# mct10/Speech-Vecalign

Measured on AMD Instinct MI355X. Metric: aligned doc-pairs/sec, higher is better.
Workload: dtype bf16; 1 GPU; synthetic 4096x4096 d=1024 bf16 embeddings, 4 overlap layers/side, 10 alignment types, band 14, coarse-to-fine (max_size_full_dp=300), 1024 doc-pairs per GPU per step; pipeline=1, N=4096, M=4096, d=1024, overlaps=4, parallelism=dp1 (pairs sharded, no collective)

## Files before the change

### speech-vecalign_amd/csrc/svx_api.hip

```cpp
#include <stdarg.h>
#include <stdio.h>
#include <stdlib.h>
#include <string.h>

#include <chrono>
#include <functional>
#include <memory>
#include <type_traits>
#include <vector>

#include "svx_common.h"

static char g_err[512] = "";

int svx_fail(svx_ctx* ctx, int code, const char* fmt, ...) {
    char* dst = ctx ? ctx->err : g_err;
    va_list ap;
    va_start(ap, fmt);
    vsnprintf(dst, 512, fmt, ap);
    va_end(ap);
    return code;
}

static const char* kStageNames[] = {"pyr0",       "pyrN",     "pyr_aux",      "knob_scoresN", "knob",      "dense_costs",
// ... 809 lines not shown
    if (bump.off > H.arena_bytes) {
        SVX_HIP(ctx, hipDeviceSynchronize());
        if (H.arena) SVX_HIP(ctx, hipFree(H.arena));
        H.arena = nullptr;
        H.arena_bytes = 0;
        const size_t want = bump.off + bump.off / 16 + (1 << 20);
        hipError_t e = hipMalloc(&H.arena, want);
        if (e != hipSuccess) return svx_fail(ctx, SVX_ERR_NOMEM, "scratch arena: hipMalloc(%zu) failed: %s", want, hipGetErrorString(e));
        H.arena_bytes = want;
    }
    const size_t desc_bytes = (size_t)n_pairs * sizeof(SvxPairDev);
    if (desc_bytes > H.pinned_cap) {
        SVX_HIP(ctx, hipDeviceSynchronize());
        if (H.pinned) SVX_HIP(ctx, hipHostFree(H.pinned));
        H.pinned = nullptr;
        H.pinned_cap = 0;
        SVX_HIP(ctx, hipHostMalloc(reinterpret_cast<void**>(&H.pinned), desc_bytes + desc_bytes / 8, hipHostMallocDefault));
        H.pinned_cap = desc_bytes + desc_bytes / 8;
    }
    char* base = H.arena;
    const char* ulo = reinterpret_cast<const char*>(1);
    const char* uhi = reinterpret_cast<const char*>(bump.off + 1);
    auto patch = [&](auto& ptr) {
        const char* v = reinterpret_cast<const char*>(ptr);
        if (v >= ulo && v < uhi) ptr = reinterpret_cast<typename std::remove_reference<decltype(ptr)>::type>(base + (v - ulo));
    };
    for (int p = 0; p < n_pairs; p++) {
        SvxPairDev& P = host[p];
        const svx_pair& in = pairs[p];
        for (int l = 0; l <= P.L; l++) {
            SvxLevel& Lv = P.lev[l];
            for (int s = 0; s < 2; s++) {
                patch(Lv.P[s]); patch(Lv.part[s]); patch(Lv.mean[s]); patch(Lv.rbar[s]); patch(Lv.inv[s]);
                if (!(l == 0 && P.norm_override[s])) patch(Lv.nrm[s]);
            }
            patch(Lv.kscore); patch(Lv.korder); patch(Lv.kys); patch(Lv.kstart);
            if (!in.del_pen) patch(Lv.pen);
            patch(Lv.path); patch(Lv.path_len); patch(Lv.cstart); patch(Lv.nchunks); patch(Lv.costs); patch(Lv.boff); patch(Lv.csum); patch(Lv.xp); patch(Lv.yp); patch(Lv.bpk);
            patch(Lv.boff_out);
            if (l > 0) { patch(Lv.align); patch(Lv.scores); patch(Lv.n_align); }
        }
        patch(P.dcost);
        patch(P.ddot);
        patch(P.dbp);
        patch(P.t_lo); patch(P.t_cnt); patch(P.t_pref); patch(P.t_flag);
    }
    H.dpairs = reinterpret_cast<SvxPairDev*>(base + o_desc);
    return SVX_OK;
}

struct Op {
    double us;
    int stage;
    std::function<int()> fn;
};

static int run_op(svx_ctx* ctx, const Op& op, hipStream_t st) {
    hipStream_t keep = ctx->stream;
    ctx->stream = st;
    int rc;
    if (op.stage < 0) {
        rc = op.fn();
    } else {
        StageScope sc(ctx, op.stage);
        rc = op.fn();
    }
    ctx->stream = keep;
    return rc;
}

static int next_event(svx_ctx* ctx, hipEvent_t* out) {
    svx_ctx_ext* cx = X(ctx);
    if (cx->ev_pool.size() < 256) {
        hipEvent_t e;
        SVX_HIP(ctx, hipEventCreateWithFlags(&e, hipEventDisableTiming));
        cx->ev_pool.push_back(e);
        *out = e;
        return SVX_OK;
    }
    *out = cx->ev_pool[cx->ev_next++ % cx->ev_pool.size()];
    return SVX_OK;
}

static void front_ops(svx_ctx* ctx, HalfState& H, std::vector<Op>& ops, int split) {
    svx_ctx_ext* cx = X(ctx);
    HalfState* h = &H;
    const BatchParams& bp = H.bp;
    const int np = H.n_pairs, d = bp.d, dtype = bp.dtype;
    const double waves = (double)((np + 1023) / 1024);
    const int parts = (split > 1 && np >= 16 * split) ? split : 1;
    struct Evs { hipEvent_t pass[SVX_MAX_LEVELS][8]; };
    auto evs = std::make_shared<Evs>();
    ops.push_back({0.0, -1, [=]() -> int {
        SVX_HIP(ctx, hipEventRecord(cx->side_fork, ctx->stream));
        SVX_HIP(ctx, hipStreamWaitEvent(cx->side, cx->side_fork, 0));
        SVX_HIP(ctx, hipStreamWaitEvent(cx->helper, cx->side_fork, 0));
        return SVX_OK;
    }});
    static const bool early_sort = getenv("SVX_SORT_EARLY") != nullptr;
    auto sort_op = [=]() -> int {
        hipStream_t main_stream = ctx->stream;
        static const bool inline_sort = getenv("SVX_SORT_INLINE") != nullptr;
        if (parts > 1 && !inline_sort && !early_sort) SVX_HIP(ctx, hipStreamWaitEvent(cx->side, evs->pass[0][parts - 1], 0));
        ctx->stream = inline_sort ? main_stream : cx->side;
        int rc;
        {
            StageScope sc(ctx, S_KNOB_SORT);
            rc = svxl_knob_scores(ctx, h->dpairs, np, h->maxL, h->max_kn, h->max_n0, dtype, d, 0);
        }
        ctx->stream = main_stream;
        if (rc) return rc;
        SVX_HIP(ctx, hipEventRecord(cx->side_join, inline_sort ? main_stream : cx->side));
        return SVX_OK;
    };
    if (parts == 1 || early_sort) ops.push_back({0.0, -1, sort_op});
    for (int l = 0; l <= H.maxL; l++) {
        for (int q = 0; q < parts; q++) {
            const int lo = (int)((long long)np * q / parts), hi = (int)((long long)np * (q + 1) / parts);
            const double aux_us = (l == 0 ? 700.0 * waves : 250.0) / parts;
            if (parts == 1) {
                ops.push_back({aux_us, S_PYR_AUX, [=]() { return svxl_pyramid_level(ctx, h->dpairs, np, l, dtype, d, h->max_nblk[l], h->max_ksum, 0); }});
                ops.push_back({H.b_pyr[l] / (l == 0 ? 4.9e6 : 5.3e6), l == 0 ? S_PYR0 : (l == 1 ? S_PYR1 : S_PYRN),
                               [=]() { return svxl_pyramid_level(ctx, h->dpairs, np, l, dtype, d, h->max_nblk[l], h->max_ksum, 1); }});
                continue;
            }
            ops.push_back({H.b_pyr[l] / (l == 0 ? 4.9e6 : 5.3e6) / parts, l == 0 ? S_PYR0 : (l == 1 ? S_PYR1 : S_PYRN), [=]() -> int {
                hipStream_t main_stream = ctx->stream;
                int rc;
                if (l == 0 && q == 0) {
                    StageScope sc(ctx, S_PYR_AUX);
                    if ((rc = svxl_pyramid_level(ctx, h->dpairs + lo, hi - lo, l, dtype, d, h->max_nblk[l], h->max_ksum, 0))) return rc;
                } else {
                    if (l > 0) SVX_HIP(ctx, hipStreamWaitEvent(cx->helper, evs->pass[l - 1][q], 0));
                    ctx->stream = cx->helper;
                    {
                        StageScope sc(ctx, S_PYR_AUX);
                        rc = svxl_pyramid_level(ctx, h->dpairs + lo, hi - lo, l, dtype, d, h->max_nblk[l], h->max_ksum, 0);
                    }
                    ctx->stream = main_stream;
                    if (rc) return rc;
                    hipEvent_t aux_done;
                    if ((rc = next_event(ctx, &aux_done))) return rc;
                    SVX_HIP(ctx, hipEventRecord(aux_done, cx->helper));
                    SVX_HIP(ctx, hipStreamWaitEvent(main_stream, aux_done, 0));
                }
                if ((rc = svxl_pyramid_level(ctx, h->dpairs + lo, hi - lo, l, dtype, d, h->max_nblk[l], h->max_ksum, 1))) return rc;
                if ((rc = next_event(ctx, &evs->pass[l][q]))) return rc;
                SVX_HIP(ctx, hipEventRecord(evs->pass[l][q], main_stream));
                return SVX_OK;
            }});
        }
        if (parts > 1 && l == 0 && !early_sort) ops.push_back({0.0, -1, sort_op});
    }
    if (!bp.straight) {
        ops.push_back({H.dense_cells * 2.7e-5, S_DENSE_COSTS, [=]() -> int {
            int rc = svxl_dense_costs_batch(ctx, h->dpairs, np, h->max_ds0, h->max_ds1, dtype, d);
            if (rc) return rc;
            return svxl_knob_from_dots(ctx, h->dpairs, np, h->max_kn);
        }});
    }
    if (H.maxL >= 1) {
        ops.push_back({H.b_knobN / 16.5e6, S_KNOB_SCORES, [=]() -> int {
            SVX_HIP(ctx, hipStreamWaitEvent(ctx->stream, cx->side_join, 0));
            return svxl_knob_scores(ctx, h->dpairs, np, h->maxL, h->max_kn, h->max_n0, dtype, d, 1);
        }});
    }
    ops.push_back({H.b_knob0 / 8.5e6, S_KNOB_SCORES0, [=]() -> int {
        SVX_HIP(ctx, hipStreamWaitEvent(ctx->stream, cx->side_join, 0));
        return svxl_knob_scores(ctx, h->dpairs, np, h->maxL, h->max_kn, h->max_n0, dtype, d, 2);
    }});
}

struct Seg {
    std::vector<Op> lb;
    bool has_s = false;
    Op s;
};

static void chain_segs(svx_ctx* ctx, HalfState& H, std::vector<Seg>& segs) {
    HalfState* h = &H;
    const BatchParams bp = H.bp;
    const int np = H.n_pairs, d = bp.d, dtype = bp.dtype, W = bp.W, B = bp.B;
    const double waves = (double)((np + 1023) / 1024);
    Seg cur;
    cur.lb.push_back({(np * (H.maxL + 1) * 0.21 < 300.0 ? 300.0 : np * (H.maxL + 1) * 0.21), S_KNOB,
                      [=]() { return svxl_del_penalty_batch(ctx, h->dpairs, np, h->maxL + 1, bp.frac); }});
    if (!bp.straight)
        cur.lb.push_back({(H.max_ds0 + H.max_ds1) * 1.7 * waves, S_DENSE_DP, [=]() { return svxl_dense_stage_batch(ctx, h->dpairs, np, h->max_ds0); }});
    const int first_depth = H.maxL > 0 ? H.maxL - 1 : 0;
    for (int depth = first_depth; depth >= 0; depth--) {
        const SvxTypes ty = depth == 0 ? bp.tfinal : bp.t11;
        int lim = 0, tamax = 0;
        if (!bp.tiles) svxl_band2_limits(ty, W, depth, dtype, d, &lim, &tamax);
        const int maxA = H.max_A[depth];
        const int src_rows = (H.maxL > 0 && !H.any_L0) ? maxA / 2 + 8 : maxA;
        cur.lb.push_back({maxA * 0.08 * waves + 60.0, depth == 0 ? S_PATH0 : S_PATH, [=]() {
            return svxl_search_path_batch(ctx, h->dpairs, np, depth, maxA, src_rows, lim, tamax);
        }});
        cur.has_s = true;
        if (bp.tiles) {
            cur.s = {1.0e4, S_TILES, [=]() {
                int* tk = reinterpret_cast<int*>(h->arena + h->o_tickets);
                float* planes = h->b_planes ? reinterpret_cast<float*>(h->arena + h->o_planes) : nullptr;
                return svxl_band_tiles_batch(ctx, h->dpairs, np, ty, W, dtype, h->max_tnd, tk, tk + (size_t)h->max_tnd * np + 1, planes);
            }};
        } else {
            cur.s = {H.b_bc[depth] / 4.0e6, depth == 0 ? S_BAND_COSTS0 : S_BAND_COSTSN, [=]() {
                return svxl_band_costs2_batch(ctx, h->dpairs, np, depth, maxA, ty, W, dtype, d);
            }};
        }
        segs.push_back(cur);
        cur = Seg();
        if (!bp.tiles)
            cur.lb.push_back({maxA * (0.21 + 0.054 * (ty.n > 1 ? ty.n : 0)) * waves, depth == 0 ? S_BAND_DP0 : S_BAND_DPN,
                              [=]() { return svxl_sparse_dp_batch(ctx, h->dpairs, np, depth, ty, B); }});
        cur.lb.push_back({maxA * 0.27 * waves, depth == 0 ? S_TRACEBACK0 : S_TRACEBACK, [=]() { return svxl_sparse_traceback_batch(ctx, h->dpairs, np, depth, B, maxA, bp.packable ? 1 : 0); }});
    }
    segs.push_back(cur);
}

static int ensure_streams(svx_ctx* ctx) {
    svx_ctx_ext* cx = X(ctx);
    if (!cx->side_ready) {
        int prio_lo = 0, prio_hi = 0;
        SVX_HIP(ctx, hipDeviceGetStreamPriorityRange(&prio_lo, &prio_hi));
        SVX_HIP(ctx, hipStreamCreateWithPriority(&cx->side, hipStreamNonBlocking, prio_lo));
        SVX_HIP(ctx, hipStreamCreateWithPriority(&cx->helper, hipStreamNonBlocking, prio_hi));
        SVX_HIP(ctx, hipEventCreateWithFlags(&cx->side_fork, hipEventDisableTiming));
        SVX_HIP(ctx, hipEventCreateWithFlags(&cx->side_join, hipEventDisableTiming));
        cx->side_ready = true;
    }
    if (!cx->chain_ready) {
        int prio_lo = 0, prio_hi = 0;
        SVX_HIP(ctx, hipDeviceGetStreamPriorityRange(&prio_lo, &prio_hi));
        SVX_HIP(ctx, hipStreamCreateWithPriority(&cx->chain, hipStreamNonBlocking, prio_hi));
        cx->chain_ready = true;
    }
    for (int h = 0; h < 2; h++) {
        if (!cx->half[h].front_done) SVX_HIP(ctx, hipEventCreateWithFlags(&cx->half[h].front_done, hipEventDisableTiming));
        if (!cx->half[h].chain_done) SVX_HIP(ctx, hipEventCreateWithFlags(&cx->half[h].chain_done, hipEventDisableTiming));
        if (!cx->half[h].upload_done) SVX_HIP(ctx, hipEventCreateWithFlags(&cx->half[h].upload_done, hipEventDisableTiming));
    }
    return SVX_OK;
}

static int run_interleaved(svx_ctx* ctx, HalfState* front, HalfState* chain, bool beside) {
    svx_ctx_ext* cx = X(ctx);
    hipStream_t A = ctx->stream, Bst = beside ? cx->chain : ctx->stream;
    std::vector<Op> fops;
    std::vector<Seg> segs;
    if (front) {
        if (front->chain_done_valid) SVX_HIP(ctx, hipStreamWaitEvent(A, front->chain_done, 0));
        {
            StageScope sc(ctx, S_SETUP);
            if (front->upload_valid) SVX_HIP(ctx, hipEventSynchronize(front->upload_done));
            memcpy(front->pinned, front->host.data(), (size_t)front->n_pairs * sizeof(SvxPairDev));
            SVX_HIP(ctx, hipMemcpyAsync(front->dpairs, front->pinned, (size_t)front->n_pairs * sizeof(SvxPairDev), hipMemcpyHostToDevice, A));
            SVX_HIP(ctx, hipEventRecord(front->upload_done, A));
            front->upload_valid = true;
            hipLaunchKernelGGL(k_init_batch, dim3(front->n_pairs), dim3(64), 0, A, front->dpairs);
            SVX_LAUNCH_CHECK(ctx, "k_init_batch");
            if (front->bp.around) {
                int rc = svxl_prior_ingest_batch(ctx, front->dpairs, front->n_pairs);
                if (rc) return rc;
            }
            if (front->bp.nsamp == 0) {
                for (int p = 0; p < front->n_pairs; p++)
                    for (int l = 0; l <= front->host[p].L; l++)
                        for (int s = 0; s < 2; s++)
                            SVX_HIP(ctx, hipMemsetAsync(front->host[p].lev[l].rbar[s], 0, (size_t)front->bp.d * sizeof(float), A));
            }
        }
        static const int split_env = [] { const char* e = getenv("SVX_PIPE_SPLIT"); const int v = e ? atoi(e) : 2; return v >= 1 && v <= 8 ? v : 2; }();
        front_ops(ctx, *front, fops, beside ? split_env : 1);
    }
    if (chain) chain_segs(ctx, *chain, segs);
    int rc;
    size_t fi = 0;
    if (chain && beside) SVX_HIP(ctx, hipStreamWaitEvent(Bst, chain->front_done, 0));
    for (size_t g = 0; g < segs.size(); g++) {
        double need = 0.0;
        for (const Op& op : segs[g].lb) {
            if ((rc = run_op(ctx, op, Bst))) return rc;
            need += op.us;
        }
        hipEvent_t lb_done = nullptr;
        if (beside) {
            if ((rc = next_event(ctx, &lb_done))) return rc;
            SVX_HIP(ctx, hipEventRecord(lb_done, Bst));
        }
        if (!segs[g].has_s) break;
        double acc = 0.0;
        need = need * 1.25 + 50.0;
        while (beside && fi < fops.size() && acc < need) {
            if ((rc = run_op(ctx, fops[fi], A))) return rc;
            acc += fops[fi].us;
            fi++;
        }
        if (beside) SVX_HIP(ctx, hipStreamWaitEvent(A, lb_done, 0));
        if ((rc = run_op(ctx, segs[g].s, A))) return rc;
        if (beside) {
            hipEvent_t s_done;
            if ((rc = next_event(ctx, &s_done))) return rc;
            SVX_HIP(ctx, hipEventRecord(s_done, A));
            SVX_HIP(ctx, hipStreamWaitEvent(Bst, s_done, 0));
        }
    }
    for (; fi < fops.size(); fi++)
        if ((rc = run_op(ctx, fops[fi], A))) return rc;
    if (front) {
        SVX_HIP(ctx, hipEventRecord(front->front_done, A));
        front->chain_pending = true;
    }
    if (chain) {
        SVX_HIP(ctx, hipEventRecord(chain->chain_done, Bst));
        chain->chain_done_valid = true;
        chain->chain_pending = false;
    }
    return SVX_OK;
}

extern "C" int svx_flush(svx_ctx* ctx) {
    if (!ctx) return SVX_ERR_ARG;
    svx_ctx_ext* cx = X(ctx);
    bool any = false;
    for (int h = 0; h < 2; h++) any = any || cx->half[h].chain_pending || cx->half[h].chain_done_valid;
    if (!any) return SVX_OK;
    SVX_HIP(ctx, hipSetDevice(ctx->device));
    int rc;
    for (int h = 0; h < 2; h++)
        if (cx->half[h].chain_pending && (rc = run_interleaved(ctx, nullptr, &cx->half[h], true))) return rc;
    for (int h = 0; h < 2; h++)
        if (cx->half[h].chain_done_valid) SVX_HIP(ctx, hipStreamWaitEvent(ctx->stream, cx->half[h].chain_done, 0));
    return SVX_OK;
}

static int align_impl(svx_ctx* ctx, const svx_align_params* prm, const svx_pair* pairs, const svx_prior* priors, int n_pairs) {
// ... 185 lines not shown
```

### speech-vecalign_amd/csrc/svx_costs.hip

```cpp
#include <stdlib.h>

#include "svx_common.h"
#include "svx_slab.h"

namespace {

constexpr int RS = 144;

template <typename E>
struct Mma;
template <>
struct Mma<ElemBF16> {
    static constexpr int KS = 64, NK = 2, KSTEP_BYTES = 64;
    using frag = uint4;
    __device__ static __forceinline__ int lane_off(int lane) { return (lane & 15) * RS + 16 * (lane >> 4); }
    __device__ static __forceinline__ frag load(const char* p) { return *reinterpret_cast<const uint4*>(p); }
    __device__ static __forceinline__ void mma(f32x4_t& acc, const frag& a, const frag& b) {
        acc = __builtin_amdgcn_mfma_f32_16x16x32_bf16(__builtin_bit_cast(bf16x8_t, a), __builtin_bit_cast(bf16x8_t, b), acc, 0, 0, 0);
    }
};
template <>
struct Mma<ElemF16> {
    static constexpr int KS = 64, NK = 2, KSTEP_BYTES = 64;
    using frag = uint4;
    __device__ static __forceinline__ int lane_off(int lane) { return (lane & 15) * RS + 16 * (lane >> 4); }
    __device__ static __forceinline__ frag load(const char* p) { return *reinterpret_cast<const uint4*>(p); }
    __device__ static __forceinline__ void mma(f32x4_t& acc, const frag& a, const frag& b) {
        acc = __builtin_amdgcn_mfma_f32_16x16x32_f16(__builtin_bit_cast(f16x8_t, a), __builtin_bit_cast(f16x8_t, b), acc, 0, 0, 0);
    }
};
template <>
struct Mma<ElemF32> {
    static constexpr int KS = 32, NK = 8, KSTEP_BYTES = 16;
    using frag = float;
    __device__ static __forceinline__ int lane_off(int lane) { return (lane & 15) * RS + 4 * (lane >> 4); }
    __device__ static __forceinline__ frag load(const char* p) { return *reinterpret_cast<const float*>(p); }
    __device__ static __forceinline__ void mma(f32x4_t& acc, const frag& a, const frag& b) {
        acc = __builtin_amdgcn_mfma_f32_16x16x4f32(a, b, acc, 0, 0, 0);
    }
};

template <typename E>
__device__ __forceinline__ void stage_slab(char* slab, const char* const* rowptr, int nrows, int k0, int d, int tid,
                                           int nthreads) {
    using S = typename E::storage;
    const int npieces = nrows * 8;
    for (int q = tid; q < npieces; q += nthreads) {
        const int r = q >> 3, p = q & 7;
        const char* ptr = rowptr[r];
        const int kel = k0 + p * E::VEC;
        uint4 v = make_uint4(0, 0, 0, 0);
        if (ptr != nullptr && kel < d) v = *reinterpret_cast<const uint4*>(ptr + (size_t)kel * sizeof(S));
        *reinterpret_cast<uint4*>(slab + r * RS + p * 16) = v;
    }
}

struct DenseArgs {
    const void* v0;
    const void* v1;
    int s0, s1, d;
    const float* inv0;
    const float* inv1;
    const float* n0;
    const float* n1;
    int mul0, mul1;
    float* costs;
    float* dots;
};

constexpr int DT = 64;
template <typename E>
__device__ void dense_block(const DenseArgs& g, int bx, int by, char* smem) {
    using S = typename E::storage;
    const int tid = threadIdx.x, lane = tid & 63, wave = tid >> 6;
    const char** rowptr = reinterpret_cast<const char**>(smem);
    char* slab = smem + 2 * DT * sizeof(char*);
    const int x0 = bx * DT, y0 = by * DT;
    if (tid < 2 * DT) {
        const int side = tid >= DT, loc = tid - side * DT;
        const int gi = (side ? y0 : x0) + loc;
        const int nn = side ? g.s1 : g.s0;
        const char* base = reinterpret_cast<const char*>(side ? g.v1 : g.v0);
        rowptr[tid] = (gi < nn) ? base + (size_t)gi * g.d * sizeof(S) : nullptr;
    }
    f32x4_t acc[2][2];
#pragma unroll
    for (int i = 0; i < 2; i++)
#pragma unroll
        for (int j = 0; j < 2; j++) acc[i][j] = (f32x4_t){0.f, 0.f, 0.f, 0.f};
    const int xt = wave >> 1, yt = wave & 1;
    for (int k0 = 0; k0 < g.d; k0 += Mma<E>::KS) {
        __syncthreads();
        stage_slab<E>(slab, rowptr, 2 * DT, k0, g.d, tid, blockDim.x);
        __syncthreads();
        const char* ap = slab + xt * 32 * RS + Mma<E>::lane_off(lane);
        const char* bp = slab + (DT + yt * 32) * RS + Mma<E>::lane_off(lane);
#pragma unroll
        for (int ks = 0; ks < Mma<E>::NK; ks++) {
            const typename Mma<E>::frag a0 = Mma<E>::load(ap + ks * Mma<E>::KSTEP_BYTES);
            const typename Mma<E>::frag a1 = Mma<E>::load(ap + 16 * RS + ks * Mma<E>::KSTEP_BYTES);
            const typename Mma<E>::frag b0 = Mma<E>::load(bp + ks * Mma<E>::KSTEP_BYTES);
            const typename Mma<E>::frag b1 = Mma<E>::load(bp + 16 * RS + ks * Mma<E>::KSTEP_BYTES);
            Mma<E>::mma(acc[0][0], a0, b0);
            Mma<E>::mma(acc[0][1], a0, b1);
            Mma<E>::mma(acc[1][0], a1, b0);
            Mma<E>::mma(acc[1][1], a1, b1);
        }
    }
#pragma unroll
    for (int i = 0; i < 2; i++)
#pragma unroll
        for (int j = 0; j < 2; j++) {
            const int y = y0 + yt * 32 + j * 16 + (lane & 15);
#pragma unroll
            for (int r = 0; r < 4; r++) {
                const int x = x0 + xt * 32 + i * 16 + (lane >> 4) * 4 + r;
                if (x < g.s0 && y < g.s1) {
                    float sumx = acc[i][j][r];
                    if (g.inv0) sumx = sumx * g.inv0[x] * g.inv1[y];
                    float c = cost_formula(sumx, 1, 1, g.n0[x], g.n1[y]);
                    c = (c * (float)g.mul0) * (float)g.mul1;
                    g.costs[(size_t)x * g.s1 + y] = c;
                    if (g.dots) g.dots[(size_t)x * g.s1 + y] = sumx;
                }
            }
        }
}

template <typename E>
__global__ __launch_bounds__(256) void k_dense_costs(DenseArgs g) {
    extern __shared__ __attribute__((aligned(16))) char smem[];
    dense_block<E>(g, blockIdx.x, blockIdx.y, smem);
}

template <typename E, bool LV0>
__global__ __launch_bounds__(256) void k_dense_costs_batch(const SvxPairDev* __restrict__ pairs) {
    extern __shared__ __attribute__((aligned(16))) char smem[];
    const SvxPairDev& P = pairs[blockIdx.z];
    if ((P.L == 0) != LV0) return;
    const SvxLevel& Lv = P.lev[P.L];
    DenseArgs g;
    g.s0 = Lv.n[0];
    g.s1 = Lv.n[1];
    if ((int)blockIdx.x * DT >= g.s0 || (int)blockIdx.y * DT >= g.s1) return;
    g.d = P.d;
    g.v0 = LV0 ? P.v[0] : (const void*)Lv.P[0];
    g.v1 = LV0 ? P.v[1] : (const void*)Lv.P[1];
    g.inv0 = LV0 ? Lv.inv[0] : nullptr;
    g.inv1 = LV0 ? Lv.inv[1] : nullptr;
    g.n0 = Lv.nrm[0];
    g.n1 = Lv.nrm[1];
    g.mul0 = 1;
    g.mul1 = 1;
    g.costs = P.dcost;
    g.dots = LV0 ? nullptr : P.ddot;
    dense_block<E>(g, blockIdx.x, blockIdx.y, smem);
}

template <typename E, int NCH>
__device__ __forceinline__ float row_dot(const typename E::storage* a, const typename E::storage* b, int d, int lane) {
    float s = 0.f;
#pragma unroll
    for (int c = 0; c < NCH; c++) {
        const int col = (c * SVX_WAVE + lane) * E::VEC;
        if (col < d) {
            float x[E::VEC], y[E::VEC];
            load_piece<E>(a + col, x);
            load_piece<E>(b + col, y);
#pragma unroll
            for (int i = 0; i < E::VEC; i++) s += x[i] * y[i];
        }
    }
    return wave_sum(s);
}

struct ScoreArgs {
    const void* v1;
    const void* v2;
    const float* inv1;
    const float* inv2;
    const float* n1;
    const float* n2;
    const int* xx;
    const int* yy;
    int64_t n;
    int rows1, rows2, d;
    float* out;
};

template <typename E, int NCH>
__device__ void score_block(const ScoreArgs& g, int64_t first, int64_t stride) {
    using S = typename E::storage;
    const int lane = threadIdx.x & 63;
    for (int64_t i = first; i < g.n; i += stride) {
        int xi = g.xx[i], yi = g.yy[i];
        xi = xi < 0 ? 0 : (xi >= g.rows1 ? g.rows1 - 1 : xi);
        yi = yi < 0 ? 0 : (yi >= g.rows2 ? g.rows2 - 1 : yi);
        float dot = row_dot<E, NCH>(reinterpret_cast<const S*>(g.v1) + (size_t)xi * g.d,
                                    reinterpret_cast<const S*>(g.v2) + (size_t)yi * g.d, g.d, lane);
        if (lane == 0) {
            if (g.inv1) dot = dot * g.inv1[xi] * g.inv2[yi];
            const float den = g.n1[xi] + g.n2[yi];
            g.out[i] = (float)((2.0 * (1.0 - (double)dot)) / (double)den);
        }
    }
}

template <typename E, int NCH>
__global__ __launch_bounds__(256) void k_score_path(ScoreArgs g) {
    score_block<E, NCH>(g, (int64_t)blockIdx.x * 4 + (threadIdx.x >> 6), (int64_t)gridDim.x * 4);
}

template <int NT>
__device__ __forceinline__ void knob_sort_block(const int* __restrict__ kx, const int* __restrict__ ky, int kn, int n, int m,
                                                int* __restrict__ korder, int* __restrict__ kys, int* __restrict__ kstart,
                                                int* cnt, int* part, size_t lds_bytes) {
    const int tid = threadIdx.x, lane = tid & 63, wave = tid >> 6;
    const bool staged = ((size_t)n + 1 + (size_t)kn) * sizeof(int) <= lds_bytes;
    int* ord = cnt + n + 1;
    for (int i = tid; i < n; i += NT) cnt[i] = 0;
    __syncthreads();
    for (int i = tid; i < kn; i += NT) {
        int x = kx[i];
        x = x < 0 ? 0 : (x >= n ? n - 1 : x);
        atomicAdd(&cnt[x], 1);
    }
    __syncthreads();
    const int per = (n + NT - 1) / NT;
    const int lo = tid * per < n ? tid * per : n, hi = (lo + per) < n ? (lo + per) : n;
    int sum = 0;
    for (int i = lo; i < hi; i++) sum += cnt[i];
    int inc = sum;
#pragma unroll
    for (int o = 1; o < 64; o <<= 1) {
        const int t = __shfl_up(inc, o, 64);
        if (lane >= o) inc += t;
    }
    if (lane == 63) part[wave] = inc;
    __syncthreads();
    int run = inc - sum;
    for (int w = 0; w < wave; w++) run += part[w];
    for (int i = lo; i < hi; i++) {
        const int v = cnt[i];
        cnt[i] = run;
        kstart[i] = run;
        run += v;
    }
    if (tid == 0) kstart[n] = kn;
    __syncthreads();
    if (staged) {
        for (int i = tid; i < kn; i += NT) {
            int x = kx[i];
            x = x < 0 ? 0 : (x >= n ? n - 1 : x);
            ord[atomicAdd(&cnt[x], 1)] = i;
        }
        __syncthreads();
        for (int p = tid; p < kn; p += NT) {
            const int i = ord[p];
            int y = ky[i];
            y = y < 0 ? 0 : (y >= m ? m - 1 : y);
            korder[p] = i;
            kys[p] = y;
        }
        return;
    }
    for (int i = tid; i < kn; i += NT) {
        int x = kx[i];
        x = x < 0 ? 0 : (x >= n ? n - 1 : x);
        const int pos = atomicAdd(&cnt[x], 1);
        int y = ky[i];
        y = y < 0 ? 0 : (y >= m ? m - 1 : y);
        korder[pos] = i;
        kys[pos] = y;
    }
}

template <int NT>
__global__ __launch_bounds__(NT) void k_knob_sort(const SvxPairDev* __restrict__ pairs, unsigned lds_bytes) {
    extern __shared__ __attribute__((aligned(16))) char smem[];
    __shared__ int part[NT / 64];
    const SvxPairDev& P = pairs[blockIdx.y];
    const int level = blockIdx.x;
    if (level > P.L) return;
    if (P.L >= 1 && level == P.L) return;
    const SvxLevel& Lv = P.lev[level];
    knob_sort_block<NT>(Lv.kx, Lv.ky, Lv.kn, Lv.n[0], Lv.n[1], Lv.korder, Lv.kys, Lv.kstart, reinterpret_cast<int*>(smem), part,
                        lds_bytes);
}

template <int NT>
__global__ __launch_bounds__(NT) void k_knob_sort_plain(const int* __restrict__ kx, const int* __restrict__ ky, int kn, int n, int m,
                                                        int* __restrict__ korder, int* __restrict__ kys, int* __restrict__ kstart,
                                                        unsigned lds_bytes) {
    extern __shared__ __attribute__((aligned(16))) char smem[];
    __shared__ int part[NT / 64];
    knob_sort_block<NT>(kx, ky, kn, n, m, korder, kys, kstart, reinterpret_cast<int*>(smem), part, lds_bytes);
}

constexpr int KNOB_PF = 2;

template <typename E, int NCH, bool LV0>
__global__ __launch_bounds__(256) void k_knob_scores(const SvxPairDev* __restrict__ pairs, int nlev, int bpt) {
    using S = typename E::storage;
    constexpr int EPL = NCH * E::VEC;
    const unsigned wg = xcd_remap(blockIdx.x, gridDim.x);
    const int task = wg / bpt, blk = wg % bpt;
    const SvxPairDev& P = pairs[task / nlev];
    const int level = task % nlev + (LV0 ? 0 : 1);
    if (level > P.L) return;
    if (!LV0 && level == P.L) return;
    const SvxLevel& Lv = P.lev[level];
    const int lane = threadIdx.x & 63;
    const int n = Lv.n[0], d = P.d;
    const S* v1 = LV0 ? reinterpret_cast<const S*>(P.v[0]) : reinterpret_cast<const S*>(Lv.P[0]);
    const S* v2 = LV0 ? reinterpret_cast<const S*>(P.v[1]) : reinterpret_cast<const S*>(Lv.P[1]);
    const float* inv1 = LV0 ? Lv.inv[0] : nullptr;
    const float* inv2 = LV0 ? Lv.inv[1] : nullptr;
    for (int x = blk * 4 + (threadIdx.x >> 6); x < n; x += bpt * 4) {
        const int s0 = gld(Lv.kstart + x), s1 = gld(Lv.kstart + x + 1);
        if (s0 >= s1) continue;
        float xr[EPL];
#pragma unroll
        for (int c = 0; c < NCH; c++) {
            const int col = (c * SVX_WAVE + lane) * E::VEC;
            if (col < d) {
                gload_piece<E>(v1 + (size_t)x * d + col, xr + c * E::VEC);
            } else {
#pragma unroll
                for (int i = 0; i < E::VEC; i++) xr[c * E::VEC + i] = 0.f;
            }
        }
        const float nx = gld(Lv.nrm[0] + x);
        const float ix = LV0 ? gld(inv1 + x) : 1.0f;
        constexpr int PF = KNOB_PF;
        const int ns = s1 - s0;
        for (int cb = 0; cb < ns; cb += SVX_WAVE) {
            const int cn = min(SVX_WAVE, ns - cb);
            const int ys_l = lane < cn ? gld(Lv.kys + s0 + cb + lane) : 0;
            const int is_l = lane < cn ? gld(Lv.korder + s0 + cb + lane) : 0;
            const float nrm_l = lane < cn ? gld(Lv.nrm[1] + ys_l) : 0.f;
            const float inv_l = (LV0 && lane < cn) ? gld(inv2 + ys_l) : 1.f;
            float dots_l = 0.f;
            uint4 yraw[PF][NCH];
#pragma unroll
            for (int u = 0; u < PF; u++) {
                const int yu = __builtin_amdgcn_readlane(ys_l, u);
#pragma unroll
                for (int c = 0; c < NCH; c++) {
                    const int col = (c * SVX_WAVE + lane) * E::VEC;
                    yraw[u][c] = (u < cn && col < d) ? gld16(v2 + (size_t)yu * d + col) : make_uint4(0, 0, 0, 0);
                }
            }
            for (int base = 0; base < cn; base += PF) {
#pragma unroll
                for (int u = 0; u < PF; u++) {
                    const int k = base + u;
                    if (k >= cn) break;
                    float dot = 0.f;
#pragma unroll
                    for (int c = 0; c < NCH; c++) {
                        float yr[E::VEC];
                        decode_piece<E>(yraw[u][c], yr);
#pragma unroll
                        for (int e = 0; e < E::VEC; e++) dot += xr[c * E::VEC + e] * yr[e];
                    }
                    if (k + PF < cn) {
                        const int yn = __builtin_amdgcn_readlane(ys_l, k + PF);
#pragma unroll
                        for (int c = 0; c < NCH; c++) {
                            const int col = (c * SVX_WAVE + lane) * E::VEC;
                            yraw[u][c] = col < d ? gld16(v2 + (size_t)yn * d + col) : make_uint4(0, 0, 0, 0);
                        }
                    }
                    dot = wave_sum(dot);
                    dots_l = lane == k ? dot : dots_l;
                }
            }
            if (lane < cn) {
                float dot = dots_l;
                if (LV0) dot = dot * ix * inv_l;
                const float den = nx + nrm_l;
                gst(Lv.kscore + is_l, (float)((2.0 * (1.0 - (double)dot)) / (double)den));
            }
        }
    }
}

template <typename E, int NCH, bool LV0>
__global__ __launch_bounds__(256) void k_knob_scores_unsorted(const SvxPairDev* __restrict__ pairs) {
    const SvxPairDev& P = pairs[blockIdx.z];
    const int level = (int)blockIdx.y + (LV0 ? 0 : 1);
    if (level > P.L) return;
    if (!LV0 && level == P.L) return;
    const SvxLevel& Lv = P.lev[level];
    ScoreArgs g;
    g.v1 = LV0 ? P.v[0] : (const void*)Lv.P[0];
    g.v2 = LV0 ? P.v[1] : (const void*)Lv.P[1];
    g.inv1 = LV0 ? Lv.inv[0] : nullptr;
    g.inv2 = LV0 ? Lv.inv[1] : nullptr;
    g.n1 = Lv.nrm[0];
    g.n2 = Lv.nrm[1];
    g.xx = Lv.kx;
    g.yy = Lv.ky;
    g.n = Lv.kn;
    g.rows1 = Lv.n[0];
    g.rows2 = Lv.n[1];
    g.d = P.d;
    g.out = Lv.kscore;
    score_block<E, NCH>(g, (int64_t)blockIdx.x * 4 + (threadIdx.x >> 6), (int64_t)gridDim.x * 4);
}

__global__ __launch_bounds__(256) void k_knob_from_dots(const SvxPairDev* __restrict__ pairs) {
    const SvxPairDev& P = pairs[blockIdx.y];
    if (P.L < 1) return;
    const SvxLevel& Lv = P.lev[P.L];
    const int n = Lv.n[0], m = Lv.n[1];
    for (int i = blockIdx.x * 256 + threadIdx.x; i < Lv.kn; i += gridDim.x * 256) {
        int x = Lv.kx[i], y = Lv.ky[i];
        x = x < 0 ? 0 : (x >= n ? n - 1 : x);
        y = y < 0 ? 0 : (y >= m ? m - 1 : y);
        const float dot = P.ddot[(size_t)x * m + y];
        const float den = Lv.nrm[0][x] + Lv.nrm[1][y];
        Lv.kscore[i] = (float)((2.0 * (1.0 - (double)dot)) / (double)den);
    }
}

inline int nch_f32(int d) {
    int c = (d + 255) / 256;
    return c <= 1 ? 1 : c <= 2 ? 2 : c <= 4 ? 4 : 8;
}
inline int nch_16(int d) {
    int c = (d + 511) / 512;
    return c <= 1 ? 1 : c <= 2 ? 2 : 4;
}

constexpr size_t DENSE_SMEM = 2 * DT * sizeof(char*) + 2 * DT * RS;

}

int svxl_dense_costs(svx_ctx* ctx, const float* v0, int s0, const float* v1, int s1, int d, const float* n0,
                     const float* n1, int mul0, int mul1, float* costs) {
    if (s0 <= 0 || s1 <= 0) return SVX_OK;
    DenseArgs g{v0, v1, s0, s1, d, nullptr, nullptr, n0, n1, mul0, mul1, costs, nullptr};
    hipLaunchKernelGGL(k_dense_costs<ElemF32>, dim3((s0 + DT - 1) / DT, (s1 + DT - 1) / DT), dim3(256), DENSE_SMEM, ctx->stream, g);
    SVX_LAUNCH_CHECK(ctx, "k_dense_costs");
    return SVX_OK;
}

int svxl_dense_costs_batch(svx_ctx* ctx, const SvxPairDev* pairs, int n_pairs, int max_s0, int max_s1, int dtype, int d) {
    (void)d;
    if (n_pairs <= 0 || max_s0 <= 0 || max_s1 <= 0) return SVX_OK;
    dim3 grid((max_s0 + DT - 1) / DT, (max_s1 + DT - 1) / DT, n_pairs);
    hipLaunchKernelGGL((k_dense_costs_batch<ElemF32, false>), grid, dim3(256), DENSE_SMEM, ctx->stream, pairs);
    if (dtype == SVX_F32)
        hipLaunchKernelGGL((k_dense_costs_batch<ElemF32, true>), grid, dim3(256), DENSE_SMEM, ctx->stream, pairs);
    else if (dtype == SVX_F16)
        hipLaunchKernelGGL((k_dense_costs_batch<ElemF16, true>), grid, dim3(256), DENSE_SMEM, ctx->stream, pairs);
    else
        hipLaunchKernelGGL((k_dense_costs_batch<ElemBF16, true>), grid, dim3(256), DENSE_SMEM, ctx->stream, pairs);
    SVX_LAUNCH_CHECK(ctx, "k_dense_costs_batch");
    return SVX_OK;
}

int svxl_score_path(svx_ctx* ctx, const int* xx, const int* yy, int64_t n, const float* n1, const float* n2,
                    const float* v1, int rows1, const float* v2, int rows2, int d, float* out) {
    if (n <= 0) return SVX_OK;
    ScoreArgs g{v1, v2, nullptr, nullptr, n1, n2, xx, yy, n, rows1, rows2, d, out};
    int64_t nb = (n + 3) / 4;
    if (nb > 16384) nb = 16384;
#define M(N) hipLaunchKernelGGL((k_score_path<ElemF32, N>), dim3((unsigned)nb), dim3(256), 0, ctx->stream, g)
    switch (nch_f32(d)) {
        case 1: M(1); break;
        case 2: M(2); break;
        case 4: M(4); break;
        default: M(8); break;
    }
#undef M
    SVX_LAUNCH_CHECK(ctx, "k_score_path");
    return SVX_OK;
}

int svxl_knob_from_dots(svx_ctx* ctx, const SvxPairDev* pairs, int n_pairs, int max_kn) {
    if (n_pairs <= 0 || max_kn <= 0) return SVX_OK;
    int nb = (max_kn + 255) / 256;
    if (nb > 16) nb = 16;
    hipLaunchKernelGGL(k_knob_from_dots, dim3(nb, n_pairs), dim3(256), 0, ctx->stream, pairs);
    SVX_LAUNCH_CHECK(ctx, "k_knob_from_dots");
    return SVX_OK;
}

constexpr size_t KNOB_SORT_HIST_LDS = 150 * 1024;
constexpr size_t KNOB_SORT_STAGE_LDS = SVX_KNOB_SORT_STAGE_LDS;
static_assert(KNOB_SORT_STAGE_LDS >= KNOB_SORT_HIST_LDS, "a launch sized for staging must still hold the longest histogram");

static size_t knob_sort_lds(int max_n0, int max_kn) {
    const size_t want = ((size_t)max_n0 + 1 + (size_t)max_kn) * sizeof(int);
    return want < KNOB_SORT_STAGE_LDS ? want : KNOB_SORT_STAGE_LDS;
}

static int knob_sort_threads() {
    static const int nt = [] {
        const char* e = getenv("SVX_SORT_THREADS");
        const int v = e ? atoi(e) : 0;
        return (v == 256 || v == 512 || v == 1024) ? v : 256;
    }();
    return nt;
}

template <int NT>
static int knob_sort_launch(svx_ctx* ctx, const SvxPairDev* pairs, int n_pairs, int max_L, size_t smem) {
    if (smem > 64 * 1024)
        SVX_HIP(ctx, hipFuncSetAttribute((const void*)k_knob_sort<NT>, hipFuncAttributeMaxDynamicSharedMemorySize, (int)smem));
    hipLaunchKernelGGL(k_knob_sort<NT>, dim3(max_L + 1, n_pairs), dim3(NT), smem, ctx->stream, pairs, (unsigned)smem);
    SVX_LAUNCH_CHECK(ctx, "k_knob_sort");
    return SVX_OK;
}

template <int NT>
static int knob_sort_plain_launch(svx_ctx* ctx, const int* kx, const int* ky, int kn, int n, int m, int* korder, int* kys,
                                  int* kstart, size_t smem) {
    if (smem > 64 * 1024)
        SVX_HIP(ctx, hipFuncSetAttribute((const void*)k_knob_sort_plain<NT>, hipFuncAttributeMaxDynamicSharedMemorySize, (int)smem));
    hipLaunchKernelGGL(k_knob_sort_plain<NT>, dim3(1), dim3(NT), smem, ctx->stream, kx, ky, kn, n, m, korder, kys, kstart,
                       (unsigned)smem);
    SVX_LAUNCH_CHECK(ctx, "k_knob_sort_plain");
    return SVX_OK;
}

int svxl_knob_sort(svx_ctx* ctx, const int* kx, const int* ky, int kn, int n, int m, int* korder, int* kys, int* kstart) {
    if ((size_t)(n + 1) * sizeof(int) > KNOB_SORT_HIST_LDS)
        return svx_fail(ctx, SVX_ERR_ARG, "knob_sort: %d source rows exceed the LDS histogram (max %d)", n,
                        (int)(KNOB_SORT_HIST_LDS / sizeof(int)) - 1);
    const size_t smem = knob_sort_lds(n, kn);
    switch (knob_sort_threads()) {
        case 256: return knob_sort_plain_launch<256>(ctx, kx, ky, kn, n, m, korder, kys, kstart, smem);
        case 512: return knob_sort_plain_launch<512>(ctx, kx, ky, kn, n, m, korder, kys, kstart, smem);
        default: return knob_sort_plain_launch<1024>(ctx, kx, ky, kn, n, m, korder, kys, kstart, smem);
    }
}

int svxl_knob_scores(svx_ctx* ctx, const SvxPairDev* pairs, int n_pairs, int max_L, int max_kn, int max_n0, int dtype, int d,
                     int part) {
    if (n_pairs <= 0 || max_kn <= 0) return SVX_OK;
    hipStream_t st = ctx->stream;
    const bool unsorted = (size_t)(max_n0 + 1) * sizeof(int) > KNOB_SORT_HIST_LDS;
    if (unsorted) {
        if (part == 0) return SVX_OK;
        const int nbu = (max_kn + 3) / 4 < 2048 ? (max_kn + 3) / 4 : 2048;
#define U32(N, LV0, GY) hipLaunchKernelGGL((k_knob_scores_unsorted<ElemF32, N, LV0>), dim3(nbu, GY, n_pairs), dim3(256), 0, st, pairs)
#define U16(E, N) hipLaunchKernelGGL((k_knob_scores_unsorted<E, N, true>), dim3(nbu, 1, n_pairs), dim3(256), 0, st, pairs)
        if (part == 1) {
            if (max_L >= 1) {
                switch (nch_f32(d)) {
                    case 1: U32(1, false, max_L); break;
                    case 2: U32(2, false, max_L); break;
                    case 4: U32(4, false, max_L); break;
                    default: U32(8, false, max_L); break;
                }
            }
        } else if (dtype == SVX_F32) {
            switch (nch_f32(d)) {
                case 1: U32(1, true, 1); break;
                case 2: U32(2, true, 1); break;
                case 4: U32(4, true, 1); break;
                default: U32(8, true, 1); break;
            }
        } else if (dtype == SVX_F16) {
            switch (nch_16(d)) {
                case 1: U16(ElemF16, 1); break;
                case 2: U16(ElemF16, 2); break;
                default: U16(ElemF16, 4); break;
            }
        } else {
            switch (nch_16(d)) {
                case 1: U16(ElemBF16, 1); break;
                case 2: U16(ElemBF16, 2); break;
                default: U16(ElemBF16, 4); break;
            }
        }
#undef U32
#undef U16
        SVX_LAUNCH_CHECK(ctx, "k_knob_scores_unsorted");
        return SVX_OK;
    }
    if (part == 0) {
        const size_t smem = knob_sort_lds(max_n0, max_kn);
        switch (knob_sort_threads()) {
            case 256: return knob_sort_launch<256>(ctx, pairs, n_pairs, max_L, smem);
            case 512: return knob_sort_launch<512>(ctx, pairs, n_pairs, max_L, smem);
            default: return knob_sort_launch<1024>(ctx, pairs, n_pairs, max_L, smem);
        }
    }
    int nb = (max_n0 + 3) / 4;
    if (nb > 1024) nb = 1024;
#define M32(N, LV0, GY) hipLaunchKernelGGL((k_knob_scores<ElemF32, N, LV0>), dim3((unsigned)nb * (GY) * n_pairs), dim3(256), 0, st, pairs, GY, nb)
#define M16(E, N) hipLaunchKernelGGL((k_knob_scores<E, N, true>), dim3((unsigned)nb * n_pairs), dim3(256), 0, st, pairs, 1, nb)
    if (part == 1 && max_L >= 1) {
        switch (nch_f32(d)) {
            case 1: M32(1, false, max_L); break;
            case 2: M32(2, false, max_L); break;
            case 4: M32(4, false, max_L); break;
            default: M32(8, false, max_L); break;
        }
    }
    if (part != 2) {
    } else if (dtype == SVX_F32) {
        switch (nch_f32(d)) {
            case 1: M32(1, true, 1); break;
            case 2: M32(2, true, 1); break;
            case 4: M32(4, true, 1); break;
            default: M32(8, true, 1); break;
        }
// ... 19 lines not shown
```

Before: 9747 doc-pairs/s.

## Run dense costs one block per pair with double-buffered slabs; move into segment chain

The batched dense-cost kernel now launches one workgroup per doc-pair instead of a 3D grid of 64x64 tiles. Each workgroup loops over all of its pair's tiles and double-buffers the K-slabs in LDS, so the next global load overlaps the current MFMA work; launch bounds allow higher occupancy. The dense-cost op is also moved out of the pyramid op list and into the per-segment chain ahead of the deletion-penalty and dense DP stages, which changes how it is scheduled. The risk is less parallelism when pairs have many tiles, and the handling of non-multiple-of-64 row and K tails is now done by hand.

```diff
diff --git a/speech-vecalign_amd/csrc/svx_api.hip b/speech-vecalign_amd/csrc/svx_api.hip
--- a/speech-vecalign_amd/csrc/svx_api.hip
+++ b/speech-vecalign_amd/csrc/svx_api.hip
@@ -985,13 +985,6 @@
         }
         if (parts > 1 && l == 0 && !early_sort) ops.push_back({0.0, -1, sort_op});
     }
-    if (!bp.straight) {
-        ops.push_back({H.dense_cells * 2.7e-5, S_DENSE_COSTS, [=]() -> int {
-            int rc = svxl_dense_costs_batch(ctx, h->dpairs, np, h->max_ds0, h->max_ds1, dtype, d);
-            if (rc) return rc;
-            return svxl_knob_from_dots(ctx, h->dpairs, np, h->max_kn);
-        }});
-    }
     if (H.maxL >= 1) {
         ops.push_back({H.b_knobN / 16.5e6, S_KNOB_SCORES, [=]() -> int {
             SVX_HIP(ctx, hipStreamWaitEvent(ctx->stream, cx->side_join, 0));
@@ -1009,6 +1002,8 @@
     bool has_s = false;
     Op s;
 };
+
+constexpr double DENSE_US_PER_CELL = 2.7e-5;
 
 static void chain_segs(svx_ctx* ctx, HalfState& H, std::vector<Seg>& segs) {
     HalfState* h = &H;
@@ -1016,6 +1011,13 @@
     const int np = H.n_pairs, d = bp.d, dtype = bp.dtype, W = bp.W, B = bp.B;
     const double waves = (double)((np + 1023) / 1024);
     Seg cur;
+    if (!bp.straight) {
+        cur.lb.push_back({H.dense_cells * DENSE_US_PER_CELL, S_DENSE_COSTS, [=]() -> int {
+            int rc = svxl_dense_costs_batch(ctx, h->dpairs, np, h->max_ds0, h->max_ds1, dtype, d);
+            if (rc) return rc;
+            return svxl_knob_from_dots(ctx, h->dpairs, np, h->max_kn);
+        }});
+    }
     cur.lb.push_back({(np * (H.maxL + 1) * 0.21 < 300.0 ? 300.0 : np * (H.maxL + 1) * 0.21), S_KNOB,
                       [=]() { return svxl_del_penalty_batch(ctx, h->dpairs, np, h->maxL + 1, bp.frac); }});
     if (!bp.straight)
diff --git a/speech-vecalign_amd/csrc/svx_costs.hip b/speech-vecalign_amd/csrc/svx_costs.hip
--- a/speech-vecalign_amd/csrc/svx_costs.hip
+++ b/speech-vecalign_amd/csrc/svx_costs.hip
@@ -67,6 +67,42 @@
     float* costs;
     float* dots;
 };
+
+__device__ __forceinline__ void dense_store(const DenseArgs& g, const f32x4_t (&acc)[2][2], int xw, int yw, int lane) {
+#pragma unroll
+    for (int i = 0; i < 2; i++)
+#pragma unroll
+        for (int j = 0; j < 2; j++) {
+            const int y = yw + j * 16 + (lane & 15);
+#pragma unroll
+            for (int r = 0; r < 4; r++) {
+                const int x = xw + i * 16 + (lane >> 4) * 4 + r;
+                if (x < g.s0 && y < g.s1) {
+                    float sumx = acc[i][j][r];
+                    if (g.inv0) sumx = sumx * g.inv0[x] * g.inv1[y];
+                    float c = cost_formula(sumx, 1, 1, g.n0[x], g.n1[y]);
+                    c = (c * (float)g.mul0) * (float)g.mul1;
+                    g.costs[(size_t)x * g.s1 + y] = c;
+                    if (g.dots) g.dots[(size_t)x * g.s1 + y] = sumx;
+                }
+            }
+        }
+}
+
+template <typename E>
+__device__ __forceinline__ void dense_slab_mma(f32x4_t (&acc)[2][2], const char* ap, const char* bp) {
+#pragma unroll
+    for (int ks = 0; ks < Mma<E>::NK; ks++) {
+        const typename Mma<E>::frag a0 = Mma<E>::load(ap + ks * Mma<E>::KSTEP_BYTES);
+        const typename Mma<E>::frag a1 = Mma<E>::load(ap + 16 * RS + ks * Mma<E>::KSTEP_BYTES);
+        const typename Mma<E>::frag b0 = Mma<E>::load(bp + ks * Mma<E>::KSTEP_BYTES);
+        const typename Mma<E>::frag b1 = Mma<E>::load(bp + 16 * RS + ks * Mma<E>::KSTEP_BYTES);
+        Mma<E>::mma(acc[0][0], a0, b0);
+        Mma<E>::mma(acc[0][1], a0, b1);
+        Mma<E>::mma(acc[1][0], a1, b0);
+        Mma<E>::mma(acc[1][1], a1, b1);
+    }
+}
 
 constexpr int DT = 64;
 template <typename E>
@@ -95,36 +131,9 @@
         __syncthreads();
         const char* ap = slab + xt * 32 * RS + Mma<E>::lane_off(lane);
         const char* bp = slab + (DT + yt * 32) * RS + Mma<E>::lane_off(lane);
-#pragma unroll
-        for (int ks = 0; ks < Mma<E>::NK; ks++) {
-            const typename Mma<E>::frag a0 = Mma<E>::load(ap + ks * Mma<E>::KSTEP_BYTES);
-            const typename Mma<E>::frag a1 = Mma<E>::load(ap + 16 * RS + ks * Mma<E>::KSTEP_BYTES);
-            const typename Mma<E>::frag b0 = Mma<E>::load(bp + ks * Mma<E>::KSTEP_BYTES);
-            const typename Mma<E>::frag b1 = Mma<E>::load(bp + 16 * RS + ks * Mma<E>::KSTEP_BYTES);
-            Mma<E>::mma(acc[0][0], a0, b0);
-            Mma<E>::mma(acc[0][1], a0, b1);
-            Mma<E>::mma(acc[1][0], a1, b0);
-            Mma<E>::mma(acc[1][1], a1, b1);
-        }
-    }
-#pragma unroll
-    for (int i = 0; i < 2; i++)
-#pragma unroll
-        for (int j = 0; j < 2; j++) {
-            const int y = y0 + yt * 32 + j * 16 + (lane & 15);
-#pragma unroll
-            for (int r = 0; r < 4; r++) {
-                const int x = x0 + xt * 32 + i * 16 + (lane >> 4) * 4 + r;
-                if (x < g.s0 && y < g.s1) {
-                    float sumx = acc[i][j][r];
-                    if (g.inv0) sumx = sumx * g.inv0[x] * g.inv1[y];
-                    float c = cost_formula(sumx, 1, 1, g.n0[x], g.n1[y]);
-                    c = (c * (float)g.mul0) * (float)g.mul1;
-                    g.costs[(size_t)x * g.s1 + y] = c;
-                    if (g.dots) g.dots[(size_t)x * g.s1 + y] = sumx;
-                }
-            }
-        }
+        dense_slab_mma<E>(acc, ap, bp);
+    }
+    dense_store(g, acc, x0 + xt * 32, y0 + yt * 32, lane);
 }
 
 template <typename E>
@@ -133,16 +142,73 @@
     dense_block<E>(g, blockIdx.x, blockIdx.y, smem);
 }
 
+typedef __attribute__((ext_vector_type(4))) unsigned u32x4_t;
+constexpr size_t DENSE_PAIR_SMEM = 2 * 2 * DT * RS;
+
+template <typename E>
+__device__ void dense_pair(const DenseArgs& g, char* smem) {
+    using S = typename E::storage;
+    constexpr int SLAB = 2 * DT * RS;
+    const int tid = threadIdx.x, lane = tid & 63, wave = __builtin_amdgcn_readfirstlane(tid >> 6);
+    const int xt = wave >> 1, yt = wave & 1;
+    const int piece = tid & 7, row0 = tid >> 3;
+    const int nk = (g.d + Mma<E>::KS - 1) / Mma<E>::KS;
+    const int ntx = (g.s0 + DT - 1) / DT, nty = (g.s1 + DT - 1) / DT;
+    const size_t rowbytes = (size_t)g.d * sizeof(S);
+    typedef __attribute__((address_space(1))) const u32x4_t* gquad_t;
+    const unsigned off = row0 * (unsigned)rowbytes + piece * 16;
+    const bool tail = (nk - 1) * Mma<E>::KS + piece * E::VEC < g.d;
+    auto load = [&](const char* xb, const char* yb, unsigned live, int k, u32x4_t (&v)[4]) {
+        const bool in = k + 1 < nk || tail;
+#pragma unroll
+        for (int i = 0; i < 4; i++) {
+            const char* base = (i < 2 ? xb : yb) + (size_t)k * 128 + (i & 1) * 32 * rowbytes;
+            v[i] = (u32x4_t){0u, 0u, 0u, 0u};
+            if (((live >> i) & 1u) && in) v[i] = *(gquad_t)(base + off);
+        }
+    };
+    auto store = [&](char* slab, const u32x4_t (&v)[4]) {
+#pragma unroll
+        for (int i = 0; i < 4; i++) *reinterpret_cast<u32x4_t*>(slab + (row0 + 32 * i) * RS + piece * 16) = v[i];
+    };
+    for (int t = 0; t < ntx * nty; t++) {
+        const int x0 = (t / nty) * DT, y0 = (t % nty) * DT;
+        const char* xb = reinterpret_cast<const char*>(g.v0) + (size_t)x0 * rowbytes;
+        const char* yb = reinterpret_cast<const char*>(g.v1) + (size_t)y0 * rowbytes;
+        const unsigned live = (x0 + row0 < g.s0 ? 1u : 0u) | (x0 + row0 + 32 < g.s0 ? 2u : 0u) | (y0 + row0 < g.s1 ? 4u : 0u) |
+                              (y0 + row0 + 32 < g.s1 ? 8u : 0u);
+        f32x4_t acc[2][2];
+#pragma unroll
+        for (int i = 0; i < 2; i++)
+#pragma unroll
+            for (int j = 0; j < 2; j++) acc[i][j] = (f32x4_t){0.f, 0.f, 0.f, 0.f};
+        u32x4_t v[4];
+        load(xb, yb, live, 0, v);
+        __syncthreads();
+        store(smem, v);
+        for (int k = 0; k < nk; k++) {
+            char* cur = smem + (k & 1) * SLAB;
+            char* nxt = smem + ((k + 1) & 1) * SLAB;
+            __syncthreads();
+            if (k + 1 < nk) load(xb, yb, live, k + 1, v);
+            dense_slab_mma<E>(acc, cur + xt * 32 * RS + Mma<E>::lane_off(lane), cur + (DT + yt * 32) * RS + Mma<E>::lane_off(lane));
+            if (k + 1 < nk) store(nxt, v);
+        }
+        int elane = lane;
+        asm volatile("" : "+v"(elane));
+        dense_store(g, acc, x0 + xt * 32, y0 + yt * 32, elane);
+    }
+}
+
 template <typename E, bool LV0>
-__global__ __launch_bounds__(256) void k_dense_costs_batch(const SvxPairDev* __restrict__ pairs) {
+__global__ __launch_bounds__(256, 8) void k_dense_costs_batch(const SvxPairDev* __restrict__ pairs) {
     extern __shared__ __attribute__((aligned(16))) char smem[];
-    const SvxPairDev& P = pairs[blockIdx.z];
+    const SvxPairDev& P = pairs[blockIdx.x];
     if ((P.L == 0) != LV0) return;
     const SvxLevel& Lv = P.lev[P.L];
     DenseArgs g;
     g.s0 = Lv.n[0];
     g.s1 = Lv.n[1];
-    if ((int)blockIdx.x * DT >= g.s0 || (int)blockIdx.y * DT >= g.s1) return;
     g.d = P.d;
     g.v0 = LV0 ? P.v[0] : (const void*)Lv.P[0];
     g.v1 = LV0 ? P.v[1] : (const void*)Lv.P[1];
@@ -154,7 +220,7 @@
     g.mul1 = 1;
     g.costs = P.dcost;
     g.dots = LV0 ? nullptr : P.ddot;
-    dense_block<E>(g, blockIdx.x, blockIdx.y, smem);
+    dense_pair<E>(g, smem);
 }
 
 template <typename E, int NCH>
@@ -450,14 +516,14 @@
 int svxl_dense_costs_batch(svx_ctx* ctx, const SvxPairDev* pairs, int n_pairs, int max_s0, int max_s1, int dtype, int d) {
     (void)d;
     if (n_pairs <= 0 || max_s0 <= 0 || max_s1 <= 0) return SVX_OK;
-    dim3 grid((max_s0 + DT - 1) / DT, (max_s1 + DT - 1) / DT, n_pairs);
-    hipLaunchKernelGGL((k_dense_costs_batch<ElemF32, false>), grid, dim3(256), DENSE_SMEM, ctx->stream, pairs);
+    const dim3 grid(n_pairs);
+    hipLaunchKernelGGL((k_dense_costs_batch<ElemF32, false>), grid, dim3(256), DENSE_PAIR_SMEM, ctx->stream, pairs);
     if (dtype == SVX_F32)
-        hipLaunchKernelGGL((k_dense_costs_batch<ElemF32, true>), grid, dim3(256), DENSE_SMEM, ctx->stream, pairs);
+        hipLaunchKernelGGL((k_dense_costs_batch<ElemF32, true>), grid, dim3(256), DENSE_PAIR_SMEM, ctx->stream, pairs);
     else if (dtype == SVX_F16)
-        hipLaunchKernelGGL((k_dense_costs_batch<ElemF16, true>), grid, dim3(256), DENSE_SMEM, ctx->stream, pairs);
+        hipLaunchKernelGGL((k_dense_costs_batch<ElemF16, true>), grid, dim3(256), DENSE_PAIR_SMEM, ctx->stream, pairs);
     else
-        hipLaunchKernelGGL((k_dense_costs_batch<ElemBF16, true>), grid, dim3(256), DENSE_SMEM, ctx->stream, pairs);
+        hipLaunchKernelGGL((k_dense_costs_batch<ElemBF16, true>), grid, dim3(256), DENSE_PAIR_SMEM, ctx->stream, pairs);
     SVX_LAUNCH_CHECK(ctx, "k_dense_costs_batch");
     return SVX_OK;
 }
```

Result: no change. 9654 doc-pairs/s (-0.9%).
